# ithewei/libhv

Hardware: AMD Instinct MI355X
Metric: device-resident WS unmask GiB/s, 64 KiB masked frames, 1/2/4/8 MI355X (higher is better)
Workload: dtype u8

## Files before the change

### include/hvws.h

```cpp
#ifndef HVWS_H
#define HVWS_H

#include <stddef.h>
#include <stdint.h>

#include "websocket_parser.h"

#ifdef __cplusplus
extern "C" {
#endif

enum {
    HVWS_OK = 0,
    HVWS_ENODEV = -1,
    HVWS_EINVAL = -2,
    HVWS_ENOMEM = -3,
    HVWS_EHIP = -4
};

#define HVWS_I_FLAGS       0xFFu
#define HVWS_I_PHASE_SHIFT 8
#define HVWS_I_HDR         (1u << 10)
#define HVWS_I_BODY        (1u << 11)
#define HVWS_I_END         (1u << 12)
// ... 291 lines not shown
#define HVWS_SUB_JOIN   1u
#define HVWS_SUB_LEAVE  2u
#define HVWS_SUB_DROP   3u
#define HVWS_SUBS_UNIQUE 1u
typedef struct hvws_sub_event { uint32_t op, topic, dest; } hvws_sub_event;
int hvws_subs_update(hvws_ctx* ctx, const uint64_t* d_topic_first, const uint32_t* d_member, uint32_t ntopics,
                     uint64_t nmember, uint32_t ndest, const hvws_sub_event* events, uint64_t nev,
                     const uint32_t* dest_of, uint32_t flags, uint64_t* d_topic_first_out, uint32_t* d_member_out,
                     uint64_t member_cap, uint64_t* out_nmember);
int64_t hvws_subs_count(hvws_ctx* ctx);
int hvws_get_subs_counts(hvws_ctx* ctx, uint64_t out[4]);

#define HVWS_SUBS_OVER 2u
int hvws_subs_update_routed(hvws_ctx* ctx, const uint64_t* d_topic_first, const uint32_t* d_member, uint64_t nmember,
                            const hvws_sub_event* events, uint64_t nev, uint32_t flags,
                            uint64_t* d_topic_first_out, uint32_t* d_member_out, uint64_t member_cap,
                            uint64_t* out_nmember);
int hvws_get_subs_merged(hvws_ctx* ctx, uint64_t out[4]);
int hvws_get_subs_events(hvws_ctx* ctx, hvws_sub_event* out, uint64_t first, uint64_t n);

uint64_t hvws_set_small_batch_limit(hvws_ctx* ctx, uint64_t bytes);

int hvws_set_door(hvws_ctx* ctx, int on);
int hvws_door_stats(hvws_ctx* ctx, uint64_t out[4]);
int hvws_door_health(uint64_t out[2]);
uint64_t hvws_set_door_idle_us(uint64_t us);
int hvws_debug_dump(int fd);
int hvws_debug_backtraces(int fd);
int hvws_door_info(hvws_ctx* ctx, uint64_t out[2]);
int hvws_door_stamps(hvws_ctx* ctx, uint64_t out[12]);

int hvws_set_small_zero_copy(hvws_ctx* ctx, int on);

int hvws_host_register(hvws_ctx* ctx, void* p, uint64_t bytes);
int hvws_host_unregister(hvws_ctx* ctx, void* p);

int hvws_rx_reads(hvws_ctx* ctx, char* const* reads, const uint64_t* lens, websocket_parser* carry, uint32_t n,
                  int unmask);

int hvws_pipeline(hvws_ctx* ctx, uint8_t* h_rx, uint64_t len, uint64_t chunk,
                  websocket_parser* carry);

typedef void (*hvws_msg_cb)(void* user, int opcode, const char* data, size_t len);
void* hvws_wsp_new(void);
void  hvws_wsp_free(void* h);
void  hvws_wsp_set_sink(void* h, hvws_msg_cb cb, void* user);
int   hvws_wsp_feed(void* h, const char* data, size_t len);
void  hvws_wsp_state(void* h, uint64_t out[8]);
int   hvws_wsp_feed_many(void* const* handles, const char* const* data, const size_t* len, int n, int* rets);

typedef struct hvws_feeder hvws_feeder;
hvws_feeder* hvws_feeder_new(void);
void hvws_feeder_free(hvws_feeder* f);
int  hvws_feeder_flush(hvws_feeder* f);
int  hvws_wsp_feeder_submit(hvws_feeder* f, void* const* handles, const char* const* data, const size_t* len, int n,
                            int* rets);

int hvws_set_thread_device(int device);
void hvws_thread_release(void);

#ifdef __cplusplus
}
#endif
#endif
```

### libhv_amd/__init__.py

```python
from __future__ import annotations

import ctypes
import os
from typing import List, Optional, Sequence, Tuple

import numpy as np

_HERE = os.path.dirname(os.path.abspath(__file__))
LIB_PATH = os.environ.get("HVWS_LIB") or os.path.join(_HERE, "libhvws.so")

WS_OP_CONTINUE, WS_OP_TEXT, WS_OP_BINARY = 0x0, 0x1, 0x2
WS_OP_CLOSE, WS_OP_PING, WS_OP_PONG = 0x8, 0x9, 0xA
WS_FIN, WS_HAS_MASK, WS_OP_MASK = 0x10, 0x20, 0x0F

I_HDR, I_BODY, I_END, I_START = 1 << 10, 1 << 11, 1 << 12, 1 << 13


class WsParser(ctypes.Structure):

    _fields_ = [
        ("state", ctypes.c_uint32),
        ("flags", ctypes.c_uint32),
        ("mask", ctypes.c_char * 4),
        ("mask_offset", ctypes.c_uint8),
# ... 301 lines not shown
    "hvws_feeder_free": (None, [ctypes.c_void_p]),
    "hvws_feeder_flush": (ctypes.c_int, [ctypes.c_void_p]),
    "hvws_wsp_feeder_submit": (
        ctypes.c_int,
        [ctypes.c_void_p, ctypes.POINTER(ctypes.c_void_p), ctypes.POINTER(ctypes.c_void_p), ctypes.POINTER(ctypes.c_size_t),
         ctypes.c_int, ctypes.POINTER(ctypes.c_int)],
    ),
    "hvws_set_thread_device": (ctypes.c_int, [ctypes.c_int]),
    "hvws_thread_release": (None, []),
    "hvws_unmask_kernel_name": (ctypes.c_char_p, []),
    "hvws_unmask_kernel_name_for": (ctypes.c_char_p, [ctypes.c_uint64]),
    "hvws_run_kernel_name": (ctypes.c_char_p, []),
    "hvws_set_spec_min": (ctypes.c_uint64, [ctypes.c_uint64]),
    "hvws_set_sieve_min": (ctypes.c_uint64, [ctypes.c_uint64]),
    "hvws_set_table_checks": (ctypes.c_int, [ctypes.c_int]),
    "hvws_last_sieve": (ctypes.c_int, [ctypes.c_void_p, ctypes.POINTER(ctypes.c_uint64)]),
    "hvws_set_sieve_windows": (None, [ctypes.c_uint64, ctypes.c_uint64, ctypes.POINTER(ctypes.c_uint64)]),
    "hvws_last_sieve_windows": (ctypes.c_int, [ctypes.c_void_p, ctypes.POINTER(ctypes.c_uint64)]),
    "hvws_build_kernel_name": (ctypes.c_char_p, []),
    "hvws_last_build_kernel": (ctypes.c_char_p, [ctypes.c_void_p]),
    "hvws_last_build_uniform": (ctypes.c_int, [ctypes.c_void_p]),
    "hvws_span_begin": (ctypes.c_int, [ctypes.c_void_p]),
    "hvws_span_end": (ctypes.c_int, [ctypes.c_void_p, ctypes.POINTER(ctypes.c_float)]),
    "hvws_set_door": (ctypes.c_int, [ctypes.c_void_p, ctypes.c_int]),
    "hvws_debug_dump": (ctypes.c_int, [ctypes.c_int]),
    "hvws_debug_backtraces": (ctypes.c_int, [ctypes.c_int]),
    "hvws_door_info": (ctypes.c_int, [ctypes.c_void_p, ctypes.POINTER(ctypes.c_uint64)]),
    "hvws_door_stats": (ctypes.c_int, [ctypes.c_void_p, ctypes.POINTER(ctypes.c_uint64)]),
    "hvws_door_health": (ctypes.c_int, [ctypes.POINTER(ctypes.c_uint64)]),
    "hvws_set_door_idle_us": (ctypes.c_uint64, [ctypes.c_uint64]),
    "hvws_door_stamps": (ctypes.c_int, [ctypes.c_void_p, ctypes.POINTER(ctypes.c_uint64)]),
    "hvws_set_small_batch_limit": (ctypes.c_uint64, [ctypes.c_void_p, ctypes.c_uint64]),
    "hvws_set_small_zero_copy": (ctypes.c_int, [ctypes.c_void_p, ctypes.c_int]),
    "hvws_set_validation": (ctypes.c_uint32, [ctypes.c_void_p, ctypes.c_uint32]),
    "hvws_set_unmask_variant": (ctypes.c_int, [ctypes.c_int]),
    "websocket_parser_init": (None, [ctypes.c_void_p]),
    "websocket_parser_settings_init": (None, [ctypes.c_void_p]),
    "websocket_parser_execute": (ctypes.c_size_t, [ctypes.c_void_p, ctypes.c_void_p, ctypes.c_void_p, ctypes.c_size_t]),
    "websocket_parser_decode": (None, [ctypes.c_void_p, ctypes.c_void_p, ctypes.c_size_t, ctypes.c_void_p]),
    "websocket_decode": (ctypes.c_uint8, [ctypes.c_void_p, ctypes.c_void_p, ctypes.c_size_t, ctypes.c_void_p, ctypes.c_uint8]),
    "websocket_calc_frame_size": (ctypes.c_size_t, [ctypes.c_uint32, ctypes.c_size_t]),
    "websocket_build_frame": (ctypes.c_size_t, [ctypes.c_void_p, ctypes.c_uint32, ctypes.c_void_p, ctypes.c_void_p, ctypes.c_size_t]),
    "ws_encode_key": (None, [ctypes.c_char_p, ctypes.c_char_p]),
    "ws_calc_frame_size": (ctypes.c_int, [ctypes.c_int, ctypes.c_bool]),
    "ws_build_frame": (
        ctypes.c_int,
        [ctypes.c_void_p, ctypes.c_void_p, ctypes.c_int, ctypes.c_void_p, ctypes.c_bool, ctypes.c_int, ctypes.c_bool],
    ),
}

CXX_SYMBOLS = (
    "_Z14hvws_feed_manyPKP15WebSocketParserPKPKcPKmiPi",
    "_Z18hvws_feeder_submitP11hvws_feederPKP15WebSocketParserPKPKcPKmiPi",
    "_ZN15WebSocketParserC1Ev",
    "_ZN15WebSocketParserD1Ev",
    "_ZN15WebSocketParser12FeedRecvDataEPKcm",
)


def lib() -> ctypes.CDLL:
    global _lib
    if _lib is not None:
        return _lib
    if not os.path.exists(LIB_PATH):
        raise RuntimeError(
            f"{LIB_PATH} is missing -- build it with `make -C libhv_amd/csrc` "
# ... 659 lines not shown
```

### libhv_amd/csrc/hvws_engine.cpp

```cpp
#include <hip/hip_ext.h>
#include <hip/hip_runtime.h>
#include <stdarg.h>
#include <stdio.h>
#include <stdlib.h>
#include <string.h>
#include <dirent.h>
#include <immintrin.h>
#include <execinfo.h>
#include <signal.h>
#include <sys/syscall.h>
#include <unistd.h>

#include <algorithm>
#include <chrono>
#include <vector>
#include <mutex>
#include <shared_mutex>
#include <atomic>

#include "hvws.h"
#include "hvws_internal.h"
#include "hvws_synth.h"

using namespace hvws;
// ... 356 lines not shown
    uint64_t sv_mean = 0;
    dbuf pipe_slot[3], pipe_segs;
    hipEvent_t pipe_ev[9] = {};
    dbuf stage;
    dbuf xor_stage;
    dbuf synth_sizes, synth_tiles, synth_bad;
    pass_u8 u8;
    pass_msg mg;
    pass_send sd;
    pass_replies rp;
    pass_fan fan;
    pass_route rt;
    pass_retain rn;
    pass_envelope en;
    pass_budget bg;
    pass_subs subs;
    pass_check ck;
    pass_tx tx;
    uint64_t scan_gen = 0;
    bool ev_build = false;
    hbuf h_small_in, h_small_out;
    hbuf h_small_done;
    uint64_t small_seq = 0;
    int small_poll = 1;
    bool small_quiet = false;
    hbuf h_feed;
    dbuf d_small_in, d_small_slots;
    uint64_t small_limit = 0;
    dbuf d_small_ctr;
    uint64_t small_ctr_base = 0;
    bool small_ctr_dirty = true;
    int small_zc = 1;
    uint64_t zc_batch = kZcBatch;
    uint32_t vmask = 0;
    uint32_t nseg = 0;
    uint64_t nfr = 0;
    uint64_t rx_len = 0;
    const uint8_t* rx = nullptr;
    bool have_scan = false;
    hipEvent_t ev[6] = {nullptr, nullptr, nullptr, nullptr, nullptr, nullptr};
    static constexpr int kTimeRing = 32;
    hipEvent_t tev[kTimeRing][4] = {};
    bool t_unmask[kTimeRing] = {};
    uint8_t t_rec[kTimeRing] = {};
    uint64_t t_seq = 0;
    int t_cur = 0;
    uint32_t t_every = 1;
    bool t_on = true;
    door_queue* door_q = nullptr;
    hbuf h_door, h_door_data, h_door_rec;
    dbuf d_door_slot;
    void* d_door_req = nullptr;
    bool door_live = false;
    bool door_wedged = false;
    bool door_broken = false;
    std::atomic<const char*> at{nullptr};
    uint64_t door_seq = 0;
    uint64_t door_epoch = 0;
    std::mutex door_m;
    int door_mode = -1;
    uint64_t door_launches = 0, door_calls = 0;
    hipEvent_t span_ev[4] = {};
    int variant = 0;
    bool nfr_known = false;
    dbuf chk;
    hbuf h_chk;
    hbuf h_readback;
    bool hcache_valid = false;
    std::vector<hvws_frame> hcache;
    std::vector<uint64_t> hfirst, hcount;
    std::vector<dcarry> hcarry;
};

namespace {
constexpr uint64_t kFastFrameBound = 1ull << 24;
constexpr uint64_t kReadbackPrefix = 1ull << 16;
constexpr uint64_t kSingleMin = 1ull << 20;
constexpr uint64_t kSlackMaxRecords = 1ull << 26;
constexpr uint64_t kSmallBatch = 64ull << 20;
constexpr uint64_t kSmallSegment = 1ull << 20;
constexpr uint64_t kSmallHostRecords = 1ull << 20;
int g_table_checks = -1;
bool table_checks() {
    if (__atomic_load_n(&g_table_checks, __ATOMIC_RELAXED) < 0) {
        const char* e = getenv("HVWS_CHECK_TABLES");
        int want = e && atoi(e) ? 1 : 0, unset = -1;
        __atomic_compare_exchange_n(&g_table_checks, &unset, want, false, __ATOMIC_RELAXED, __ATOMIC_RELAXED);
    }
    return __atomic_load_n(&g_table_checks, __ATOMIC_RELAXED) > 0;
}
}

namespace {

dframes frames_of(hvws_ctx* c) {
    tset& t = c->T();
    return {t.f_hdr.as<int64_t>(), t.f_off.as<uint64_t>(), t.f_len.as<uint64_t>(), t.f_length.as<uint64_t>(),
            t.f_key.as<uint32_t>(), t.f_keyrot.as<uint32_t>(), t.f_info.as<uint32_t>(), t.frame_cap};
}

hipError_t ensure_frames(hvws_ctx* c, uint64_t n, bool exact = false) {
    if (n <= c->T().frame_cap && c->T().f_off.p) return hipSuccess;
    uint64_t want = std::max<uint64_t>(exact ? n : n + n / 4, 1024);
    hipError_t e;
    tset& t = c->T();
    for (dbuf* b : {&t.f_hdr, &t.f_off, &t.f_len, &t.f_length})
        if ((e = b->ensure(want * 8)) != hipSuccess) return e;
    for (dbuf* b : {&t.f_key, &t.f_keyrot, &t.f_info})
        if ((e = b->ensure(want * 4)) != hipSuccess) return e;
    t.frame_cap = want;
    return hipSuccess;
}

void to_dcarry(const websocket_parser& p, dcarry& d) {
// ... 852 lines not shown
    if (!ho_d || !hp_d) return set_err(HVWS_EHIP, "pinned buffers not device-mapped");
    HIP_OR(c->d_small_ctr.ensure(64), HVWS_ENOMEM);
    unsigned long long* ctr = c->d_small_ctr.as<unsigned long long>();
    if (c->small_ctr_dirty) {
        HIP_OR(hipMemsetAsync(ctr, 0, 8, c->stream), HVWS_EHIP);
        c->small_ctr_base = 0;
        c->small_ctr_dirty = false;
    }
    const uint64_t ctr_base = c->small_ctr_base;
    c->small_ctr_dirty = true;
    uint8_t* d = hp_d;
    if (!zc) {
        d = c->d_small_in.as<uint8_t>();
        HIP_OR(hipMemcpyAsync(d, hp, pkt, hipMemcpyHostToDevice, c->stream), HVWS_EHIP);
        if (user_mapped && len)
            HIP_OR(hipMemcpyAsync(d + o_data, h_rx, len, hipMemcpyHostToDevice, c->stream), HVWS_EHIP);
    }
    const uint8_t* d_rx = zc ? (user_mapped ? user_mapped : hp_d + o_data) : d + o_data;
    static const bool timed_env = experiment("step_events") && atoi(experiment("step_events")) >= 2;
    const bool timed = timed_env && c->t_on;
    uint64_t* done_d = nullptr;
    const volatile uint64_t* done_h = nullptr;
    const uint64_t seq = ++c->small_seq;
    if (c->small_poll) {
        HIP_OR(c->h_small_done.ensure((uint64_t)nseg * 8 + 64), HVWS_ENOMEM);
        done_d = mapped<uint64_t>(c->h_small_done);
        done_h = c->h_small_done.as<uint64_t>();
        if (!done_d) return set_err(HVWS_EHIP, "pinned completion words not device-mapped");
    }
    HIP_OR(begin_timed_scan(c, false), HVWS_EHIP);
    HIP_OR(launch_small(d_rx, len, (const dseg*)(d + o_segs), (const dcarry*)(d + o_carry), nseg,
                        (const uint64_t*)(d + o_slot), c->d_small_slots.as<drec>(), ctr, ctr_base,
                        (drec*)(ho_d + nseg), hcap, ho_d, user_mapped ? user_mapped : hp_d + o_data, unmask,
                        c->vmask, stage_lds, done_d, seq, c->stream, timed ? c->tev[c->t_cur][0] : nullptr,
                        timed ? c->tev[c->t_cur][1] : nullptr),
           HVWS_EHIP);
    if (timed) c->t_rec[c->t_cur] |= 3u;
    if (done_h) {
        uint32_t s = 0, spins = 0;
        auto next_query = std::chrono::steady_clock::now() + std::chrono::microseconds(100);
        while (s < nseg) {
            if (done_h[s] == seq) {
                ++s;
                continue;
            }
            if ((++spins & 63u) == 0 && std::chrono::steady_clock::now() >= next_query) {
                next_query = std::chrono::steady_clock::now() + std::chrono::microseconds(100);
                const hipError_t q = hipStreamQuery(c->stream);
                if (q == hipSuccess) {
                    if (done_h[s] != seq) return set_err(HVWS_EHIP, "k_small finished without completing segment %u", s);
                    continue;
                }
                if (q != hipErrorNotReady) return set_err(HVWS_EHIP, "k_small: %s", hipGetErrorString(q));
            }
            __builtin_ia32_pause();
        }
        __atomic_thread_fence(__ATOMIC_ACQUIRE);
    } else {
        HIP_OR(hipStreamSynchronize(c->stream), HVWS_EHIP);
    }
    c->small_quiet = true;
    if (!user_mapped && unmask && len) par_memcpy(h_rx, hp + o_data, len);
    uint64_t total = 0;
    for (uint32_t s = 0; s < nseg; ++s) total += ho[s].count;
    c->small_ctr_base = ctr_base + total;
    c->small_ctr_dirty = false;
    c->hcache.resize(total);
    c->hfirst.resize(nseg);
// ... 528 lines not shown
const char* qname(hipError_t q) {
    return q == hipSuccess ? "idle" : q == hipErrorNotReady ? "busy" : hipGetErrorString(q);
}

}

extern "C" {

int hvws_debug_dump(int fd) {
    std::vector<hvws_ctx*> all;
    {
        std::lock_guard<std::mutex> lk(g_ctx_m);
        all = g_ctx_all;
    }
    dprintf(fd, "libhvws: %zu contexts, %d with a worker stream; holding %llu device bytes, %llu pinned bytes\n",
            all.size(), g_door_count.load(), (unsigned long long)g_dev_bytes.load(),
            (unsigned long long)g_pin_bytes.load());
    for (hvws_ctx* c : all) {
        dprintf(fd, "  ctx %p dev %d door_mode %d door_live %d door_seq %llu epoch %llu launches %llu calls %llu",
                (void*)c, c->device, c->door_mode, (int)c->door_live, (unsigned long long)c->door_seq,
                (unsigned long long)c->door_epoch, (unsigned long long)c->door_launches,
                (unsigned long long)c->door_calls);
        if (c->h_door.p) {
            const ddoor* b = c->h_door.as<ddoor>();
            dprintf(fd, " | mailbox%s seq %llu done %llu alive %llu exited %llu served %llu op %u",
                    c->d_door_req ? " (request in device memory)" : "",
                    (unsigned long long)__atomic_load_n(&door_req(c)->seq, __ATOMIC_ACQUIRE),
                    (unsigned long long)__atomic_load_n(&b->done, __ATOMIC_ACQUIRE),
                    (unsigned long long)__atomic_load_n(&b->alive, __ATOMIC_ACQUIRE),
                    (unsigned long long)__atomic_load_n(&b->exited, __ATOMIC_ACQUIRE),
                    (unsigned long long)__atomic_load_n(&b->served, __ATOMIC_ACQUIRE), door_req(c)->op);
        }
        const char* at = c->at.load();
        dprintf(fd, " | wedged %d broken %d | in %s | last scan path %d, have_scan %d\n", (int)c->door_wedged,
                (int)c->door_broken, at ? at : "-", c->scan_path, (int)c->have_scan);
    }
    dprintf(fd, "libhvws: worker launches wedged %llu, requests unanswered %llu (process)\n",
            (unsigned long long)g_door_wedged.load(), (unsigned long long)g_door_failed.load());
    for (hvws_ctx* c : all) {
        if (c->at.load()) {
            dprintf(fd, "  ctx %p streams: not queried (in %s)\n", (void*)c, c->at.load());
            continue;
        }
        dprintf(fd, "  ctx %p streams:", (void*)c);
        const struct {
            const char* n;
            hipStream_t s;
        } ss[] = {{"stream", c->stream}, {"sstream", c->sstream}, {"copy_in", c->copy_in},
                  {"copy_out", c->copy_out}};
        for (const auto& x : ss)
            if (x.s) dprintf(fd, " %s=%s", x.n, qname(hipStreamQuery(x.s)));
        if (c->door_q)
            dprintf(fd, " worker-queue=%s error=0x%x", door_queue_idle(c->door_q) ? "idle" : "running",
                    door_queue_error(c->door_q));
        dprintf(fd, "\n");
    }
    return (int)all.size();
}

int hvws_debug_backtraces(int fd) {
    struct sigaction sa = {}, old = {};
    sa.sa_handler = bt_handler;
    sigemptyset(&sa.sa_mask);
    sa.sa_flags = SA_RESTART;
    void* warm[4];
    (void)backtrace(warm, 4);
    g_bt_fd = fd;
    if (sigaction(SIGUSR2, &sa, &old) != 0) return -1;
// ... 35 lines not shown
    HIP_OR(hipGetDevice(&d), HVWS_EHIP);
    if (cur) *cur = d;
    HIP_OR(hipDeviceGetPCIBusId(bus_id, len, d), HVWS_EHIP);
    return HVWS_OK;
}

hvws_ctx* hvws_ctx_create(int device) {
    int n = 0;
    hipError_t e = hipGetDeviceCount(&n);
    if (e != hipSuccess || n <= 0) {
        set_err(HVWS_ENODEV, "no HIP device available (%s)", e != hipSuccess ? hipGetErrorString(e) : "count 0");
        return nullptr;
    }
    if (device < 0 || device >= n) {
        set_err(HVWS_EINVAL, "device %d out of range (have %d)", device, n);
        return nullptr;
    }
    if ((e = hipSetDevice(device)) != hipSuccess) {
        set_err(HVWS_EHIP, "hipSetDevice(%d): %s", device, hipGetErrorString(e));
        return nullptr;
    }
    hvws_ctx* c = new hvws_ctx();
    c->device = device;
    {
        std::lock_guard<std::mutex> lk(g_ctx_m);
        g_ctx_all.push_back(c);
    }
    for (hbuf& b : c->h_up) b.flags = hipHostMallocCoherent;
    c->h_status.flags = hipHostMallocCoherent;
    c->h_small_done.flags = hipHostMallocCoherent;
    if (const char* sp = experiment("small_poll")) c->small_poll = atoi(sp) ? 1 : 0;
    if (const char* zc = experiment("small_zc")) c->small_zc = atoi(zc) ? 1 : 0;
    if (const char* zb = experiment("zc_batch")) c->zc_batch = strtoull(zb, nullptr, 0);
    if (const char* sp = experiment("spec")) c->spec_mode = atoi(sp) == 0 ? 0 : (atoi(sp) == 1 ? 1 : (atoi(sp) == 2 ? 2 : -1));
    if (const char* wv = experiment("walk_verify")) c->verify_mode = atoi(wv) < 0 ? -1 : (atoi(wv) ? 1 : 0);
    int prio_least = 0, prio_greatest = 0;
    (void)hipDeviceGetStreamPriorityRange(&prio_least, &prio_greatest);
    const int scan_prio = prio_greatest;
    if (hipStreamCreateWithFlags(&c->stream, hipStreamNonBlocking) != hipSuccess ||
        hipStreamCreateWithFlags(&c->copy_in, hipStreamNonBlocking) != hipSuccess ||
        hipStreamCreateWithFlags(&c->copy_out, hipStreamNonBlocking) != hipSuccess ||
        hipStreamCreateWithPriority(&c->sstream, hipStreamNonBlocking, scan_prio) != hipSuccess) {
        set_err(HVWS_EHIP, "stream creation failed");
        hvws_ctx_destroy(c);
        return nullptr;
    }
    bool ev_ok = true;
    for (auto& ev : c->ev) ev_ok = ev_ok && hipEventCreate(&ev) == hipSuccess;
    for (auto& row : c->tev)
        for (auto& ev : row) ev_ok = ev_ok && hipEventCreate(&ev) == hipSuccess;
    for (auto& ev : c->up_ev) ev_ok = ev_ok && hipEventCreateWithFlags(&ev, hipEventDisableTiming) == hipSuccess;
    for (tset& t : c->ts) ev_ok = ev_ok && hipEventCreateWithFlags(&t.free_ev, hipEventDisableTiming) == hipSuccess;
    ev_ok = ev_ok && hipEventCreateWithFlags(&c->scan_done, hipEventDisableTiming) == hipSuccess;
    c->cs = c->stream;
    if (!ev_ok) {
        set_err(HVWS_EHIP, "event creation failed");
        hvws_ctx_destroy(c);
        return nullptr;
    }
    return c;
}

void hvws_ctx_destroy(hvws_ctx* c) {
    if (!c) return;
    hipSetDevice(c->device);
    door_release(c);
// ... 2108 lines not shown
}

int hvws_door_health(uint64_t out[2]) {
    if (!out) return set_err(HVWS_EINVAL, "null output");
    out[0] = g_door_wedged.load();
    out[1] = g_door_failed.load();
    return HVWS_OK;
}

int hvws_door_stats(hvws_ctx* c, uint64_t out[4]) {
    if (!c) c = hvws::thread_ctx();
    if (!out) return set_err(HVWS_EINVAL, "null output");
    out[0] = c->door_launches;
    out[1] = c->door_calls;
    out[2] = c->h_door.p ? __atomic_load_n(&c->h_door.as<ddoor>()->served, __ATOMIC_ACQUIRE) : 0;
    out[3] = c->door_live ? 1 : 0;
    return HVWS_OK;
}

uint64_t hvws_set_small_batch_limit(hvws_ctx* c, uint64_t bytes) {
    if (!c) c = hvws::thread_ctx();
    const uint64_t old = c->small_limit ? c->small_limit : kSmallBatch;
    c->small_limit = bytes;
    return old;
}

int hvws_set_small_zero_copy(hvws_ctx* c, int on) {
    if (!c) c = hvws::thread_ctx();
    const int old = c->small_zc;
    c->small_zc = on ? 1 : 0;
    return old;
}

const char* hvws_unmask_kernel_name(void) { return unmask_name(unmask_variant()); }

const char* hvws_unmask_kernel_name_for(uint64_t rx_len) { return unmask_name(unmask_variant_for(rx_len)); }

const char* hvws_run_kernel_name(void) { return run_kernel_name(); }

uint64_t hvws_set_spec_min(uint64_t frames) { return set_spec_min(frames); }

uint64_t hvws_set_sieve_min(uint64_t bytes) { return set_sieve_min(bytes); }

int hvws_set_table_checks(int on) {
    const int prev = table_checks() ? 1 : 0;
    __atomic_store_n(&g_table_checks, on ? 1 : 0, __ATOMIC_RELAXED);
    return prev;
}

int hvws_last_sieve(hvws_ctx* c, uint64_t out[4]) {
    if (!c) c = thread_ctx();
    if (!c || !out) return set_err(HVWS_EINVAL, "hvws_last_sieve: NULL argument");
    out[0] = out[1] = out[2] = out[3] = 0;
    if (!c->sv_ran) return HVWS_OK;
    HIP_OR(hipSetDevice(c->device), HVWS_EHIP);
    HIP_OR(hipStreamSynchronize(c->cs), HVWS_EHIP);
    const dsieve* d = c->h_sv.as<dsieve>();
    const uint64_t* n = reinterpret_cast<const uint64_t*>(c->h_sv.as<uint8_t>() + sizeof(dsieve));
    out[0] = d->active ? (n[3] <= c->sv_cap && n[0] <= c->sv_capc ? 1 : 2) : 0;
    out[1] = d->active ? n[0] : 0;
    out[2] = d->use ? d->npath : 0;
    out[3] = d->use ? d->pend : 0;
    return HVWS_OK;
}

void hvws_set_sieve_windows(uint64_t hops, uint64_t window_bytes, uint64_t prev[2]) {
// ... 79 lines not shown
}

struct thread_door_guard {
    ~thread_door_guard() {
        if (!t_ctx || !t_ctx->door_live) return;
        std::lock_guard<std::mutex> cl(t_ctx->door_m);
        if ((pid_t)syscall(SYS_gettid) == getpid()) {
            door_quit_nohip(t_ctx);
        } else {
            hipSetDevice(t_ctx->device);
            door_park(t_ctx);
        }
    }
};
thread_local thread_door_guard t_door_guard;

hvws_ctx* thread_ctx() {
    if (t_ctx) return t_ctx;
    (void)&t_door_guard;
    int dev = t_device;
    if (dev < 0) {
        const char* e = getenv("HVWS_DEVICE");
        dev = e ? atoi(e) : 0;
    }
    t_ctx = hvws_ctx_create(dev);
    if (!t_ctx) fatal("cannot open a HIP device context");
    return t_ctx;
}

void ctx_copy_settings(hvws_ctx* dst, const hvws_ctx* src) {
    dst->small_limit = src->small_limit;
    dst->small_zc = src->small_zc;
    dst->zc_batch = src->zc_batch;
    dst->vmask = src->vmask;
}

bool take_frames(hvws_ctx* c, std::vector<hvws_frame>& frames, std::vector<uint64_t>& first,
                 std::vector<uint64_t>& count) {
    if (!c->have_scan || !c->hcache_valid || c->rx) return false;
    frames.swap(c->hcache);
    first.swap(c->hfirst);
    count.swap(c->hcount);
    c->hcache.clear();
    c->hcache_valid = false;
    c->have_scan = false;
    return true;
}

bool is_pinned(const void* p, uint64_t len) { return pinned_dev(p, len) != nullptr; }

char* pinned_stage(uint64_t bytes) {
    hvws_ctx* c = thread_ctx();
    if (hipSetDevice(c->device) != hipSuccess || c->h_feed.ensure(bytes + 64) != hipSuccess)
        fatal("pinned staging allocation");
    return c->h_feed.as<char>();
}

void gpu_xor_host(char* dst, const char* src, size_t n, uint32_t key, uint32_t phase) {
    if (n == 0) return;
    hvws_ctx* c = thread_ctx();
    if (door_xor(c, dst, src, n, key, phase)) return;
    if (hipSetDevice(c->device) != hipSuccess) fatal("hipSetDevice");
    if (c->xor_stage.ensure(n + 64) != hipSuccess) fatal("device staging allocation");
    uint8_t* d = c->xor_stage.as<uint8_t>();
    if (hipMemcpyAsync(d, src, n, hipMemcpyHostToDevice, c->stream) != hipSuccess ||
        launch_xor_span(d, n, key, phase, c->stream) != hipSuccess ||
// ... 27 lines not shown
```

### libhv_amd/csrc/hvws_internal.h

```cpp
#pragma once

#include <hip/hip_runtime.h>
#include <hsa/hsa.h>
#include <stddef.h>
#include <stdlib.h>
#include <stdint.h>
#include <string.h>

#include <atomic>
#include <functional>

#include "websocket_parser.h"

struct hvws_ctx;

namespace hvws {

inline const char* experiment(const char* name) {
    const char* e = getenv("HVWS_EXPERIMENT");
    if (!e) return nullptr;
    const size_t n = strlen(name);
    for (const char* p = e; p && *p; p = strchr(p, ',') ? strchr(p, ',') + 1 : nullptr)
        if (!strncmp(p, name, n) && p[n] == '=') return p + n + 1;
    return nullptr;
// ... 210 lines not shown
    uint32_t  lgP;
};
uint64_t sieve_tiles_max(uint64_t rx_len);
uint64_t sieve_slot_words(uint64_t rx_len);
uint64_t sieve_min();
uint64_t set_sieve_min(uint64_t v);
uint64_t sieve_generation();
void sieve_geometry(uint64_t rx_len, uint64_t nframes, uint32_t& rt, uint32_t& wt);
void set_sieve_windows(uint64_t hops, uint64_t window, uint64_t prev[2]);
uint64_t sieve_hops();
hipError_t launch_sieve(const uint8_t* rx, uint64_t rx_len, const dseg* segs, const dmid* mid, const uint64_t* npred,
                        const sieve_bufs& b, hipStream_t st);
hipError_t launch_sieve_emit(const uint8_t* rx, uint64_t rx_len, const dseg* segs, const dmid* mid,
                             const sieve_bufs& b, dframes fr, uint32_t vmask, hipStream_t st);

enum scan_pass { SCAN_COUNT = 0, SCAN_EMIT = 1, SCAN_SINGLE = 2, SCAN_SPEC = 3, SCAN_SLACK = 4, SCAN_RUN = 5 };
hipError_t launch_scan(int pass, const uint8_t* rx, uint64_t rx_len, const dseg* segs, uint32_t nseg,
                       const dcarry* carry_in, dcarry* carry_out, uint64_t* counts, uint64_t* bases,
                       uint64_t* total, scan_scratch sc, dframes fr, uint32_t vmask, hipStream_t st);
hipError_t launch_offsets(const uint64_t* counts, uint64_t* bases, uint32_t nseg, uint64_t* total,
                          hipStream_t st);
hipError_t launch_publish_tiles(dspec_status* status, uint64_t seq, hipStream_t st);
hipError_t launch_cap_check(uint64_t* total, uint64_t cap, dspec_status* status, uint64_t seq, hipStream_t st);
hipError_t launch_ends_check(const uint64_t* off, const uint64_t* len, const uint64_t* nfr_dev,
                             unsigned long long* bad, hipStream_t st);
hipError_t launch_tile_index(const uint64_t* off, const uint64_t* len, uint64_t nfr, const uint64_t* nfr_dev,
                             uint32_t* tile_first, uint64_t ntiles, uint64_t tile, hipStream_t st);
constexpr uint32_t TILE_MARK = 0xFFFFFFFFu;
constexpr uint64_t TILE_SPAN_MAX = 64;
hipError_t launch_tile_fixup(const uint64_t* off, const uint64_t* len, uint64_t nfr, uint32_t* tile_first,
                             uint64_t ntiles, uint64_t tile, hipStream_t st);
constexpr uint64_t kStageSegment = 32ull << 10;
constexpr uint64_t kZcBatch = 1ull << 20;
hipError_t launch_small(const uint8_t* rx, uint64_t rx_len, const dseg* segs, const dcarry* carry_in, uint32_t nseg,
                        const uint64_t* slot_base, drec* slots, unsigned long long* rec_total, uint64_t rec_base,
                        drec* h_rec, uint64_t h_rec_cap, dsmall_out* h_out, uint8_t* h_rx, int unmask, uint32_t vmask,
                        uint32_t stage_lds, uint64_t* h_done, uint64_t seq, hipStream_t st,
                        hipEvent_t ev_start = nullptr, hipEvent_t ev_stop = nullptr);
enum : uint32_t { DOOR_FEED = 1u, DOOR_XOR = 2u, DOOR_EXIT = 3u };
constexpr uint32_t kDoorThreads = 512;
constexpr uint64_t kDoorMax = 32ull << 10;
constexpr uint64_t kDoorRecords = kDoorMax / 2 + 3;
struct ddoor {
    uint64_t seq;
    uint32_t op;
    uint32_t unmask;
    uint64_t len;
    uint32_t vmask;
    uint32_t key;
    uint32_t phase;
    uint32_t pad0;
    dcarry   carry;
    uint64_t pad1[4];
    uint64_t seq_tail;
    uint64_t done;
    uint64_t alive;
    uint64_t count;
    uint64_t served;
    dcarry   out;
    uint64_t exited;
    uint64_t pad2[1];
    uint64_t stamp[12];
};
static_assert(sizeof(dcarry) == 48, "dcarry layout");
static_assert(offsetof(ddoor, done) == 128, "ddoor: device fields on their own lines");
static_assert(offsetof(ddoor, seq_tail) == 120, "k_door reads seq_tail as the last 8 bytes of the request block");
static_assert(offsetof(ddoor, carry) == 40 && offsetof(ddoor, len) == 16 && offsetof(ddoor, vmask) == 24,
              "k_door reads the request as words 1-10");
struct door_args {
    const ddoor* req;
// ... 385 lines not shown
```

### libhv_amd/csrc/hvws_kernels.hip

```cpp
#include <stdio.h>
#include <stdlib.h>

#include <hip/hip_ext.h>

#include "hvws_dev.h"

namespace hvws {

__device__ bool scalar_frame(const uint8_t* seg, uint64_t L, dcarry& st, uint64_t& pos, frec& r, uint32_t vmask) {
    r.hdr_off = -1;
    r.pay_off = 0;
    r.pay_len = 0;
    r.length = 0;
    r.key = 0;
    r.info = 0;
    bool have = false;
    if (st.state == S_START) {
        if (pos >= L) return false;
        uint32_t b0 = seg[pos];
        st.offset = 0;
        st.length = 0;
        st.mask_offset = 0;
        st.flags = (b0 & F_OPMASK) | ((b0 & 0x80u) ? F_FIN : 0u);
        st.viol = ((b0 & 0x70u) ? V_RSV : 0u) | (reserved_opcode(b0 & F_OPMASK) ? V_OPCODE : 0u);
// ... 682 lines not shown
            } else {
                for (uint32_t b = 0; b < 16; ++b) {
                    const uint64_t x = c + b;
                    if (x >= sb && x < se) lds[x - sb16] ^= (uint8_t)((b < 8 ? mlo >> (8 * b) : mhi >> (8 * (b - 8))) & 0xFFu);
                }
            }
        } else if (whole) {
            u32x4 v = *reinterpret_cast<const u32x4*>(src + c);
            *reinterpret_cast<u32x4*>(h_rx + c) = v ^ m4;
        } else {
            for (uint32_t b = 0; b < 16; ++b) {
                const uint64_t x = c + b;
                const uint32_t kb = (uint32_t)((b < 8 ? mlo >> (8 * b) : mhi >> (8 * (b - 8))) & 0xFFu);
                if (x >= sb && x < se && kb) h_rx[x] = src[x] ^ (uint8_t)kb;
            }
        }
    }
    if (!STAGE) return;
    i = 0;
    for (uint64_t c = sb16 + (uint64_t)lane * 16u; c < se; c += 64u * 16u, ++i) {
        if (!((changed >> i) & 1u)) continue;
        if (c >= sb && c + 16 <= se) {
            *reinterpret_cast<u32x4*>(h_rx + c) = *reinterpret_cast<const u32x4*>(lds + (c - sb16));
        } else {
            for (uint32_t b = 0; b < 16; ++b) {
                const uint64_t x = c + b;
                if (x >= sb && x < se) h_rx[x] = lds[x - sb16];
            }
        }
    }
}

template <bool STAGE>
__global__ __launch_bounds__(64) void k_small(const uint8_t* __restrict__ rx, uint64_t rx_len,
                                              const dseg* __restrict__ segs, const dcarry* __restrict__ carry_in,
                                              const uint64_t* __restrict__ slot_base, drec* __restrict__ slots,
                                              unsigned long long* __restrict__ rec_total, drec* __restrict__ h_rec,
                                              uint64_t h_rec_cap, dsmall_out* __restrict__ h_out,
                                              uint8_t* __restrict__ h_rx, int unmask, uint32_t vmask,
                                              uint64_t rec_base, uint64_t* __restrict__ h_done, uint64_t seq) {
    extern __shared__ u32x4 lds_seg[];
    __shared__ drec lrec[SMALL_LREC];
    const uint32_t s = blockIdx.x;
    const uint32_t lane = threadIdx.x;
    const dseg sg = segs[s];
    dcarry st = carry_in[s];
    drec* slot = slots + slot_base[s];
    const uint64_t sb = sg.off, L = sg.len, se = sb + L;

    const uint8_t* src = rx;
    uint64_t src_len = rx_len;
    uint8_t* lds = reinterpret_cast<uint8_t*>(lds_seg);
    const uint64_t sb16 = sb & ~15ull;
    if (STAGE) {
        constexpr int SB = 8;
        for (uint64_t c0 = sb16 + (uint64_t)lane * 16u; c0 < se; c0 += 64u * 16u * SB) {
            u32x4 v[SB];
#pragma unroll
            for (int u = 0; u < SB; ++u) {
                const uint64_t c = c0 + (uint64_t)u * 1024u;
                v[u] = c >= sb && c + 16 <= se ? *reinterpret_cast<const u32x4*>(rx + c) : u32x4{0u, 0u, 0u, 0u};
            }
#pragma unroll
            for (int u = 0; u < SB; ++u) {
                const uint64_t c = c0 + (uint64_t)u * 1024u;
                if (c >= sb && c + 16 <= se) *reinterpret_cast<u32x4*>(lds + (c - sb16)) = v[u];
            }
        }
        const uint64_t c_last = (se - 1) & ~15ull;
        const uint64_t ce = lane == 0 ? sb16 : c_last;
        const bool partial = L && lane < 2 && (lane == 0 || c_last != sb16) && (ce < sb || ce + 16 > se);
        if (partial) {
            uint8_t b16[16];
#pragma unroll
            for (int b = 0; b < 16; ++b) b16[b] = ce + b >= sb && ce + b < se ? rx[ce + b] : 0;
#pragma unroll
            for (int b = 0; b < 16; ++b)
                if (ce + b >= sb && ce + b < se) lds[ce + b - sb16] = b16[b];
        }
        __syncthreads();
        src = lds - sb16;
        src_len = se;
    }

    st.started = 0;
// ... 25 lines not shown

    if (unmask && n) {
        if (n <= SMALL_LREC) {
            small_xor<STAGE>([&](uint64_t i) { return lrec[i]; }, n, sb, se, src, lds, h_rx);
        } else {
            for (uint64_t i = lane; i < SMALL_LREC; i += 64) slot[i] = lrec[i];
            __threadfence_block();
            __syncthreads();
            small_xor<STAGE>([&](uint64_t i) { return slot[i]; }, n, sb, se, src, lds, h_rx);
        }
    }

    base = __shfl(base, 0);
    const uint64_t nl = n < SMALL_LREC ? n : SMALL_LREC;
    if (base + n <= h_rec_cap) {
        for (uint64_t i = lane; i < nl; i += 64) h_rec[base + i] = lrec[i];
        for (uint64_t i = SMALL_LREC + lane; i < n; i += 64) h_rec[base + i] = slot[i];
    } else if (!(unmask && n > SMALL_LREC)) {
        for (uint64_t i = lane; i < nl; i += 64) slot[i] = lrec[i];
    }
    if (lane == 0) {
        dsmall_out o;
        o.first = base;
        o.count = n;
        o.st = st;
        h_out[s] = o;
    }
    if (h_done) {
        __threadfence_system();
        if (lane == 0) __hip_atomic_store(h_done + s, seq, __ATOMIC_RELAXED, __HIP_MEMORY_SCOPE_SYSTEM);
    }
}

hipError_t launch_small(const uint8_t* rx, uint64_t rx_len, const dseg* segs, const dcarry* carry_in, uint32_t nseg,
                        const uint64_t* slot_base, drec* slots, unsigned long long* rec_total, uint64_t rec_base,
                        drec* h_rec, uint64_t h_rec_cap, dsmall_out* h_out, uint8_t* h_rx, int unmask, uint32_t vmask,
                        uint32_t stage_lds, uint64_t* h_done, uint64_t seq, hipStream_t st, hipEvent_t ev_start,
                        hipEvent_t ev_stop) {
    if (nseg == 0) return hipSuccess;
    const bool ev = ev_start || ev_stop;
    if (stage_lds && ev)
        hipExtLaunchKernelGGL(k_small<true>, dim3(nseg), dim3(64), stage_lds, st, ev_start, ev_stop, 0u, rx, rx_len,
                              segs, carry_in, slot_base, slots, rec_total, h_rec, h_rec_cap, h_out, h_rx, unmask, vmask,
                              rec_base, h_done, seq);
    else if (stage_lds)
        hipLaunchKernelGGL(k_small<true>, dim3(nseg), dim3(64), stage_lds, st, rx, rx_len, segs, carry_in, slot_base,
                           slots, rec_total, h_rec, h_rec_cap, h_out, h_rx, unmask, vmask, rec_base, h_done, seq);
    else if (ev)
        hipExtLaunchKernelGGL(k_small<false>, dim3(nseg), dim3(64), 0, st, ev_start, ev_stop, 0u, rx, rx_len, segs,
                              carry_in, slot_base, slots, rec_total, h_rec, h_rec_cap, h_out, h_rx, unmask, vmask,
                              rec_base, h_done, seq);
    else
        hipLaunchKernelGGL(k_small<false>, dim3(nseg), dim3(64), 0, st, rx, rx_len, segs, carry_in, slot_base, slots,
                           rec_total, h_rec, h_rec_cap, h_out, h_rx, unmask, vmask, rec_base, h_done, seq);
    return hipGetLastError();
}


__device__ __forceinline__ void lds_hdr16(const uint32_t* l, uint32_t q, uint64_t& lo, uint64_t& hi) {
    const uint32_t w = q >> 2, r = q & 3u;
    const uint32_t d0 = l[w], d1 = l[w + 1], d2 = l[w + 2], d3 = l[w + 3], d4 = l[w + 4];
    const uint32_t c0 = __builtin_amdgcn_alignbyte(d1, d0, r), c1 = __builtin_amdgcn_alignbyte(d2, d1, r);
    const uint32_t c2 = __builtin_amdgcn_alignbyte(d3, d2, r), c3 = __builtin_amdgcn_alignbyte(d4, d3, r);
    lo = (uint64_t)c0 | ((uint64_t)c1 << 32);
    hi = (uint64_t)c2 | ((uint64_t)c3 << 32);
}

__device__ __forceinline__ void door_size(const uint32_t* l, uint32_t q, uint32_t& hl, uint32_t& len) {
    const uint32_t w = q >> 2, r = q & 3u;
    const uint32_t d0 = l[w], d1 = l[w + 1];
    const uint32_t b0 = __builtin_amdgcn_alignbyte(d1, d0, r);
    const uint32_t len7 = (b0 >> 8) & 0x7Fu, m4 = (b0 >> 13) & 4u;
    if (len7 < 126) {
        hl = 2u + m4;
        len = len7;
    } else if (len7 == 126) {
        hl = 4u + m4;
        len = ((b0 >> 8) & 0xFF00u) | (b0 >> 24);
    } else {
        const uint32_t d2 = l[w + 2], d3 = l[w + 3];
        const uint32_t b1 = __builtin_amdgcn_alignbyte(d2, d1, r), b2 = __builtin_amdgcn_alignbyte(d3, d2, r);
        const uint64_t be = (uint64_t)(b0 >> 16) | ((uint64_t)b1 << 16) | ((uint64_t)(b2 & 0xFFFFu) << 48);
        const uint64_t len64 = __builtin_bswap64(be);
        hl = 10u + m4;
        len = len64 > 0xFFFFFFFFull ? 0xFFFFFFFFu : (uint32_t)len64;
    }
}
// ... 1695 lines not shown
```

Measured before the change: 3007.

## Make small-segment kernel a capped persistent grid with prefetched segment metadata

Turns k_small from one block per segment into a grid-stride persistent kernel capped at 128 blocks by default. Each block loops over segments and loads the next segment's descriptor, carry and slot base before processing the current one. This is meant to cut block launch and scheduling overhead and hide metadata load latency. In exchange, a grid of 128 single-wave blocks may underfill the GPU's compute units and leave bandwidth unused when there are many segments. A runtime setter and an experiment knob for the cap are added.

```diff
diff --git a/include/hvws.h b/include/hvws.h
--- a/include/hvws.h
+++ b/include/hvws.h
@@ -347,6 +347,8 @@
 
 int hvws_set_small_zero_copy(hvws_ctx* ctx, int on);
 
+uint32_t hvws_set_small_grid(hvws_ctx* ctx, uint32_t n);
+
 int hvws_host_register(hvws_ctx* ctx, void* p, uint64_t bytes);
 int hvws_host_unregister(hvws_ctx* ctx, void* p);
 
diff --git a/libhv_amd/__init__.py b/libhv_amd/__init__.py
--- a/libhv_amd/__init__.py
+++ b/libhv_amd/__init__.py
@@ -357,6 +357,7 @@
     "hvws_door_stamps": (ctypes.c_int, [ctypes.c_void_p, ctypes.POINTER(ctypes.c_uint64)]),
     "hvws_set_small_batch_limit": (ctypes.c_uint64, [ctypes.c_void_p, ctypes.c_uint64]),
     "hvws_set_small_zero_copy": (ctypes.c_int, [ctypes.c_void_p, ctypes.c_int]),
+    "hvws_set_small_grid": (ctypes.c_uint32, [ctypes.c_void_p, ctypes.c_uint32]),
     "hvws_set_validation": (ctypes.c_uint32, [ctypes.c_void_p, ctypes.c_uint32]),
     "hvws_set_unmask_variant": (ctypes.c_int, [ctypes.c_int]),
     "websocket_parser_init": (None, [ctypes.c_void_p]),
diff --git a/libhv_amd/csrc/hvws_engine.cpp b/libhv_amd/csrc/hvws_engine.cpp
--- a/libhv_amd/csrc/hvws_engine.cpp
+++ b/libhv_amd/csrc/hvws_engine.cpp
@@ -412,6 +412,7 @@
     bool small_ctr_dirty = true;
     int small_zc = 1;
     uint64_t zc_batch = kZcBatch;
+    uint32_t small_grid = 0;
     uint32_t vmask = 0;
     uint32_t nseg = 0;
     uint64_t nfr = 0;
@@ -460,6 +461,7 @@
 constexpr uint64_t kSmallBatch = 64ull << 20;
 constexpr uint64_t kSmallSegment = 1ull << 20;
 constexpr uint64_t kSmallHostRecords = 1ull << 20;
+std::atomic<uint32_t> g_small_grid{0};
 int g_table_checks = -1;
 bool table_checks() {
     if (__atomic_load_n(&g_table_checks, __ATOMIC_RELAXED) < 0) {
@@ -1378,8 +1380,8 @@
     HIP_OR(launch_small(d_rx, len, (const dseg*)(d + o_segs), (const dcarry*)(d + o_carry), nseg,
                         (const uint64_t*)(d + o_slot), c->d_small_slots.as<drec>(), ctr, ctr_base,
                         (drec*)(ho_d + nseg), hcap, ho_d, user_mapped ? user_mapped : hp_d + o_data, unmask,
-                        c->vmask, stage_lds, done_d, seq, c->stream, timed ? c->tev[c->t_cur][0] : nullptr,
-                        timed ? c->tev[c->t_cur][1] : nullptr),
+                        c->vmask, stage_lds, c->small_grid, done_d, seq, c->stream,
+                        timed ? c->tev[c->t_cur][0] : nullptr, timed ? c->tev[c->t_cur][1] : nullptr),
            HVWS_EHIP);
     if (timed) c->t_rec[c->t_cur] |= 3u;
     if (done_h) {
@@ -1974,8 +1976,9 @@
                     (unsigned long long)__atomic_load_n(&b->served, __ATOMIC_ACQUIRE), door_req(c)->op);
         }
         const char* at = c->at.load();
-        dprintf(fd, " | wedged %d broken %d | in %s | last scan path %d, have_scan %d\n", (int)c->door_wedged,
-                (int)c->door_broken, at ? at : "-", c->scan_path, (int)c->have_scan);
+        dprintf(fd, " | wedged %d broken %d | in %s | last scan path %d, have_scan %d | small_grid %u\n",
+                (int)c->door_wedged, (int)c->door_broken, at ? at : "-", c->scan_path, (int)c->have_scan,
+                c->small_grid);
     }
     dprintf(fd, "libhvws: worker launches wedged %llu, requests unanswered %llu (process)\n",
             (unsigned long long)g_door_wedged.load(), (unsigned long long)g_door_failed.load());
@@ -2077,6 +2080,8 @@
     if (const char* sp = experiment("small_poll")) c->small_poll = atoi(sp) ? 1 : 0;
     if (const char* zc = experiment("small_zc")) c->small_zc = atoi(zc) ? 1 : 0;
     if (const char* zb = experiment("zc_batch")) c->zc_batch = strtoull(zb, nullptr, 0);
+    if (const char* sg = experiment("small_grid")) c->small_grid = (uint32_t)strtoul(sg, nullptr, 0);
+    if (const uint32_t g = g_small_grid.load(std::memory_order_relaxed)) c->small_grid = g;
     if (const char* sp = experiment("spec")) c->spec_mode = atoi(sp) == 0 ? 0 : (atoi(sp) == 1 ? 1 : (atoi(sp) == 2 ? 2 : -1));
     if (const char* wv = experiment("walk_verify")) c->verify_mode = atoi(wv) < 0 ? -1 : (atoi(wv) ? 1 : 0);
     int prio_least = 0, prio_greatest = 0;
@@ -4251,6 +4256,22 @@
     return old;
 }
 
+uint32_t hvws_set_small_grid(hvws_ctx* c, uint32_t n) {
+    if (c) {
+        const uint32_t old = c->small_grid;
+        c->small_grid = n;
+        return old;
+    }
+    const uint32_t old = g_small_grid.exchange(n, std::memory_order_relaxed);
+    if (n) {
+        hvws::thread_ctx()->small_grid = n;
+    } else {
+        const char* sg = experiment("small_grid");
+        hvws::thread_ctx()->small_grid = sg ? (uint32_t)strtoul(sg, nullptr, 0) : 0;
+    }
+    return old;
+}
+
 const char* hvws_unmask_kernel_name(void) { return unmask_name(unmask_variant()); }
 
 const char* hvws_unmask_kernel_name_for(uint64_t rx_len) { return unmask_name(unmask_variant_for(rx_len)); }
@@ -4396,6 +4417,7 @@
     dst->small_limit = src->small_limit;
     dst->small_zc = src->small_zc;
     dst->zc_batch = src->zc_batch;
+    dst->small_grid = src->small_grid;
     dst->vmask = src->vmask;
 }
 
diff --git a/libhv_amd/csrc/hvws_internal.h b/libhv_amd/csrc/hvws_internal.h
--- a/libhv_amd/csrc/hvws_internal.h
+++ b/libhv_amd/csrc/hvws_internal.h
@@ -266,10 +266,11 @@
                              uint64_t ntiles, uint64_t tile, hipStream_t st);
 constexpr uint64_t kStageSegment = 32ull << 10;
 constexpr uint64_t kZcBatch = 1ull << 20;
+constexpr uint32_t kSmallGrid = 128;
 hipError_t launch_small(const uint8_t* rx, uint64_t rx_len, const dseg* segs, const dcarry* carry_in, uint32_t nseg,
                         const uint64_t* slot_base, drec* slots, unsigned long long* rec_total, uint64_t rec_base,
                         drec* h_rec, uint64_t h_rec_cap, dsmall_out* h_out, uint8_t* h_rx, int unmask, uint32_t vmask,
-                        uint32_t stage_lds, uint64_t* h_done, uint64_t seq, hipStream_t st,
+                        uint32_t stage_lds, uint32_t grid_cap, uint64_t* h_done, uint64_t seq, hipStream_t st,
                         hipEvent_t ev_start = nullptr, hipEvent_t ev_stop = nullptr);
 enum : uint32_t { DOOR_FEED = 1u, DOOR_XOR = 2u, DOOR_EXIT = 3u };
 constexpr uint32_t kDoorThreads = 512;
diff --git a/libhv_amd/csrc/hvws_kernels.hip b/libhv_amd/csrc/hvws_kernels.hip
--- a/libhv_amd/csrc/hvws_kernels.hip
+++ b/libhv_amd/csrc/hvws_kernels.hip
@@ -738,25 +738,18 @@
 }
 
 template <bool STAGE>
-__global__ __launch_bounds__(64) void k_small(const uint8_t* __restrict__ rx, uint64_t rx_len,
-                                              const dseg* __restrict__ segs, const dcarry* __restrict__ carry_in,
-                                              const uint64_t* __restrict__ slot_base, drec* __restrict__ slots,
-                                              unsigned long long* __restrict__ rec_total, drec* __restrict__ h_rec,
-                                              uint64_t h_rec_cap, dsmall_out* __restrict__ h_out,
-                                              uint8_t* __restrict__ h_rx, int unmask, uint32_t vmask,
-                                              uint64_t rec_base, uint64_t* __restrict__ h_done, uint64_t seq) {
-    extern __shared__ u32x4 lds_seg[];
-    __shared__ drec lrec[SMALL_LREC];
-    const uint32_t s = blockIdx.x;
+__device__ __forceinline__ void small_segment(const uint32_t s, const dseg sg, dcarry st, drec* __restrict__ slot,
+                                              uint8_t* lds, drec* lrec, const uint8_t* __restrict__ rx,
+                                              uint64_t rx_len, unsigned long long* __restrict__ rec_total,
+                                              drec* __restrict__ h_rec, uint64_t h_rec_cap,
+                                              dsmall_out* __restrict__ h_out, uint8_t* __restrict__ h_rx, int unmask,
+                                              uint32_t vmask, uint64_t rec_base, uint64_t* __restrict__ h_done,
+                                              uint64_t seq) {
     const uint32_t lane = threadIdx.x;
-    const dseg sg = segs[s];
-    dcarry st = carry_in[s];
-    drec* slot = slots + slot_base[s];
     const uint64_t sb = sg.off, L = sg.len, se = sb + L;
 
     const uint8_t* src = rx;
     uint64_t src_len = rx_len;
-    uint8_t* lds = reinterpret_cast<uint8_t*>(lds_seg);
     const uint64_t sb16 = sb & ~15ull;
     if (STAGE) {
         constexpr int SB = 8;
@@ -848,27 +841,68 @@
     }
 }
 
+template <bool STAGE>
+__global__ __launch_bounds__(64) void k_small(const uint8_t* __restrict__ rx, uint64_t rx_len,
+                                              const dseg* __restrict__ segs, const dcarry* __restrict__ carry_in,
+                                              uint32_t nseg, const uint64_t* __restrict__ slot_base,
+                                              drec* __restrict__ slots, unsigned long long* __restrict__ rec_total,
+                                              drec* __restrict__ h_rec, uint64_t h_rec_cap,
+                                              dsmall_out* __restrict__ h_out, uint8_t* __restrict__ h_rx, int unmask,
+                                              uint32_t vmask, uint64_t rec_base, uint64_t* __restrict__ h_done,
+                                              uint64_t seq) {
+    extern __shared__ u32x4 lds_seg[];
+    __shared__ drec lrec[SMALL_LREC];
+    uint8_t* lds = reinterpret_cast<uint8_t*>(lds_seg);
+    uint32_t s = blockIdx.x;
+    if (s >= nseg) return;
+    dseg sg = segs[s];
+    dcarry st = carry_in[s];
+    uint64_t sl = slot_base[s];
+    for (;;) {
+        const uint32_t s_next = s + gridDim.x;
+        const bool more = s_next < nseg && s_next > s;
+        dseg sg_next = sg;
+        dcarry st_next = st;
+        uint64_t sl_next = sl;
+        if (more) {
+            sg_next = segs[s_next];
+            st_next = carry_in[s_next];
+            sl_next = slot_base[s_next];
+        }
+        small_segment<STAGE>(s, sg, st, slots + sl, lds, lrec, rx, rx_len, rec_total, h_rec, h_rec_cap, h_out, h_rx,
+                             unmask, vmask, rec_base, h_done, seq);
+        if (!more) break;
+        __syncthreads();
+        s = s_next;
+        sg = sg_next;
+        st = st_next;
+        sl = sl_next;
+    }
+}
+
 hipError_t launch_small(const uint8_t* rx, uint64_t rx_len, const dseg* segs, const dcarry* carry_in, uint32_t nseg,
                         const uint64_t* slot_base, drec* slots, unsigned long long* rec_total, uint64_t rec_base,
                         drec* h_rec, uint64_t h_rec_cap, dsmall_out* h_out, uint8_t* h_rx, int unmask, uint32_t vmask,
-                        uint32_t stage_lds, uint64_t* h_done, uint64_t seq, hipStream_t st, hipEvent_t ev_start,
-                        hipEvent_t ev_stop) {
+                        uint32_t stage_lds, uint32_t grid_cap, uint64_t* h_done, uint64_t seq, hipStream_t st,
+                        hipEvent_t ev_start, hipEvent_t ev_stop) {
     if (nseg == 0) return hipSuccess;
+    const uint32_t grid = std::min(nseg, grid_cap ? grid_cap : kSmallGrid);
     const bool ev = ev_start || ev_stop;
     if (stage_lds && ev)
-        hipExtLaunchKernelGGL(k_small<true>, dim3(nseg), dim3(64), stage_lds, st, ev_start, ev_stop, 0u, rx, rx_len,
-                              segs, carry_in, slot_base, slots, rec_total, h_rec, h_rec_cap, h_out, h_rx, unmask, vmask,
-                              rec_base, h_done, seq);
+        hipExtLaunchKernelGGL(k_small<true>, dim3(grid), dim3(64), stage_lds, st, ev_start, ev_stop, 0u, rx, rx_len,
+                              segs, carry_in, nseg, slot_base, slots, rec_total, h_rec, h_rec_cap, h_out, h_rx, unmask,
+                              vmask, rec_base, h_done, seq);
     else if (stage_lds)
-        hipLaunchKernelGGL(k_small<true>, dim3(nseg), dim3(64), stage_lds, st, rx, rx_len, segs, carry_in, slot_base,
-                           slots, rec_total, h_rec, h_rec_cap, h_out, h_rx, unmask, vmask, rec_base, h_done, seq);
+        hipLaunchKernelGGL(k_small<true>, dim3(grid), dim3(64), stage_lds, st, rx, rx_len, segs, carry_in, nseg,
+                           slot_base, slots, rec_total, h_rec, h_rec_cap, h_out, h_rx, unmask, vmask, rec_base, h_done,
+                           seq);
     else if (ev)
-        hipExtLaunchKernelGGL(k_small<false>, dim3(nseg), dim3(64), 0, st, ev_start, ev_stop, 0u, rx, rx_len, segs,
-                              carry_in, slot_base, slots, rec_total, h_rec, h_rec_cap, h_out, h_rx, unmask, vmask,
+        hipExtLaunchKernelGGL(k_small<false>, dim3(grid), dim3(64), 0, st, ev_start, ev_stop, 0u, rx, rx_len, segs,
+                              carry_in, nseg, slot_base, slots, rec_total, h_rec, h_rec_cap, h_out, h_rx, unmask, vmask,
                               rec_base, h_done, seq);
     else
-        hipLaunchKernelGGL(k_small<false>, dim3(nseg), dim3(64), 0, st, rx, rx_len, segs, carry_in, slot_base, slots,
-                           rec_total, h_rec, h_rec_cap, h_out, h_rx, unmask, vmask, rec_base, h_done, seq);
+        hipLaunchKernelGGL(k_small<false>, dim3(grid), dim3(64), 0, st, rx, rx_len, segs, carry_in, nseg, slot_base,
+                           slots, rec_total, h_rec, h_rec_cap, h_out, h_rx, unmask, vmask, rec_base, h_done, seq);
     return hipGetLastError();
 }
 
```

New measurement: 3006. About the same (-0.0%).
